# gyhandy/Neural-Sim-NeRF

Measured on AMD Instinct MI355X. Metric: Mray-samples/sec at 400x400, 64+128 samples, 8x256 MLP, higher is better.
Workload: dtype f16x2

## Files before the change

neural_sim_nerf_amd/csrc/nsr_h2.inc:

```
constexpr int kStreamSlabsH2Bwd = 146;


typedef _Float16 f16x8 __attribute__((ext_vector_type(8)));
typedef _Float16 f16x2 __attribute__((ext_vector_type(2)));
typedef float f32x2 __attribute__((ext_vector_type(2)));

struct H2 { u32x4 hi, lo; };

constexpr float kH2Max = 65504.0f * (1.0f - 1.0f / 4096.0f);

struct H2Job {
  float xa, xb, m;
  unsigned hi;
  float ra, rb;
};
__device__ __forceinline__ void h2_stage0(H2Job& q) {
  asm("v_fma_mixlo_f16 %0, %1, %2, 0" : "=v"(q.hi) : "v"(q.xa), "v"(q.m));
}
__device__ __forceinline__ void h2_stage1(H2Job& q, float& amax) {
  asm("v_fma_mixhi_f16 %0, %1, %2, 0" : "+v"(q.hi) : "v"(q.xb), "v"(q.m));
  asm("v_max3_f32 %0, %0, |%1|, |%2|" : "+v"(amax) : "v"(q.xa), "v"(q.xb));
}
__device__ __forceinline__ void h2_stage2(H2Job& q) {
  asm("v_fma_mix_f32 %0, %1, %2, -%3 op_sel:[0,0,0] op_sel_hi:[0,0,1]" : "=v"(q.ra) : "v"(q.xa), "v"(q.m), "v"(q.hi));
  asm("v_fma_mix_f32 %0, %1, %2, -%3 op_sel:[0,0,1] op_sel_hi:[0,0,1]" : "=v"(q.rb) : "v"(q.xb), "v"(q.m), "v"(q.hi));
}
__device__ __forceinline__ void h2_stage3(const H2Job& q, int j, H2& r) {
  const f16x2 lo = __builtin_convertvector(f32x2{q.ra, q.rb}, f16x2);
  r.hi[j] = q.hi;
  r.lo[j] = __builtin_bit_cast(unsigned, lo);
}
__device__ __forceinline__ void split_pair_h2(float xa, float xb, float m, int j, H2& r, float& amax) {
  H2Job q{xa, xb, m, 0u, 0.0f, 0.0f};
  h2_stage0(q); h2_stage1(q, amax); h2_stage2(q); h2_stage3(q, j, r);
}

__device__ __forceinline__ f32x16 mfma_h2(f32x4 a, u32x4 b, f32x16 c) {
  return __builtin_amdgcn_mfma_f32_32x32x16_f16(__builtin_bit_cast(f16x8, a), __builtin_bit_cast(f16x8, b), c, 0, 0, 0);
}

template <int C0>
__device__ __forceinline__ void ring_issue_dma(Ring& rg) {
  char* l = rg.smem + rg.pslot * kSlabBytes + rg.wave_lds;
  const int soff = rg.pnet_off + rg.pslab * kSlabBytes;
#ifndef NSR_EXP_NODMA
  __builtin_amdgcn_raw_ptr_buffer_load_lds(rg.rsrc, (__attribute__((address_space(3))) void*)l, 16, rg.lane_off, soff,
                                           C0 * 1024, 0);
  __builtin_amdgcn_raw_ptr_buffer_load_lds(rg.rsrc, (__attribute__((address_space(3))) void*)l, 16, rg.lane_off, soff,
                                           (C0 + 1) * 1024, 0);
#endif
}
template <int C>
__device__ __forceinline__ void ring_issue_dma1(Ring& rg) {
  char* l = rg.smem + rg.pslot * kSlabBytes + rg.wave_lds;
  const int soff = rg.pnet_off + rg.pslab * kSlabBytes;
#ifndef NSR_EXP_NODMA
  __builtin_amdgcn_raw_ptr_buffer_load_lds(rg.rsrc, (__attribute__((address_space(3))) void*)l, 16, rg.lane_off, soff,
                                           C * 1024, 0);
#endif
}
template <int NS, int SLABS, int SLABS_BWD>
__device__ __forceinline__ void ring_issue_advance(Ring& rg) {
  rg.pslot = (rg.pslot + 1 == NS) ? 0 : rg.pslot + 1;
  const int nslab = rg.pslab + 1;
  const bool wrap = nslab == ((SLABS_BWD != SLABS && rg.pphase >= rg.pn1) ? SLABS_BWD : SLABS);
  rg.pslab = wrap ? 0 : nslab;
  const int nphase = (rg.pphase + 1 == rg.ppi) ? 0 : rg.pphase + 1;
  rg.pphase = wrap ? nphase : rg.pphase;
  const int net = rg.pphase < rg.pn0 ? 0 : (rg.pphase < rg.pn1 ? 1 : 2);
  rg.pnet_off = net * (int)rg.stride;
}

template <int NS, int SLABS, int SLABS_BWD>
__device__ __forceinline__ bool ring_issue_advance_a(Ring& rg) {
  rg.pslot = (rg.pslot + 1 == NS) ? 0 : rg.pslot + 1;
  const int nslab = rg.pslab + 1;
  const bool wrap = nslab == ((SLABS_BWD != SLABS && rg.pphase >= rg.pn1) ? SLABS_BWD : SLABS);
  rg.pslab = wrap ? 0 : nslab;
  return wrap;
}
__device__ __forceinline__ void ring_issue_advance_b(Ring& rg, bool wrap) {
  const int nphase = (rg.pphase + 1 == rg.ppi) ? 0 : rg.pphase + 1;
  rg.pphase = wrap ? nphase : rg.pphase;
  const int net = rg.pphase < rg.pn0 ? 0 : (rg.pphase < rg.pn1 ? 1 : 2);
  rg.pnet_off = net * (int)rg.stride;
}

template <int NS, int G, int NP, bool ACT_, bool ZH = false, bool ZL = false, int NACC>
__device__ __forceinline__ void step_h2(Ring& rg, f32x4 (&Acur)[4], f32x4 (&Anxt)[4], const H2& b, f32x16 (&acc)[NACC],
                                        int HB, int LB , int lane, H2Job (&job)[NP], int j0,
                                        H2& bn, float& amax) {
  const char* p = rg.smem + rg.cslot * kSlabBytes + (G + 1) * kStepBytes + lane * 16;
#ifdef NSR_EXP_H2_NOSPLIT
  constexpr bool ACT = false;
  if (ACT_) { bn = b; }
#else
  constexpr bool ACT = ACT_;
#endif
#ifdef NSR_EXP_H2_NOFRAG
#define NSR_H2_FRAG(i, off) do { } while (0)
#else
#define NSR_H2_FRAG(i, off) Anxt[i] = *(const f32x4*)(p + (off))
#endif
#ifdef NSR_EXP_NODMA
#define NSR_H2_DMA(C) do { } while (0)
#define NSR_H2_DMA1(C) do { } while (0)
#else
#define NSR_H2_DMA(C) ring_issue_dma<C>(rg)
#define NSR_H2_DMA1(C) ring_issue_dma1<C>(rg)
#endif
  const char* pn = nullptr;
  NSR_PIN();
  acc[HB] = mfma_h2(Acur[0], b.lo, ZH ? f32x16{0} : acc[HB]);
  NSR_PIN();
  if (G != 3) NSR_H2_FRAG(0, 0);
#if NSR_H2_SCHED == 3
  else NSR_H2_DMA1(3);
#endif
  if (ACT) for (int u = 0; u < NP; ++u) h2_stage0(job[u]);
  NSR_PIN();
  acc[HB + 1] = mfma_h2(Acur[1], b.lo, ZH ? f32x16{0} : acc[HB + 1]);
  NSR_PIN();
  if (G != 3) NSR_H2_FRAG(1, 1024);
  if (ACT) for (int u = 0; u < NP; ++u) h2_stage1(job[u], amax);
  if (G == 3) {
    NSR_PIN();
#ifdef NSR_EXP_NOVMWAIT
    asm volatile("s_waitcnt lgkmcnt(0)" ::: "memory");
#else
    asm volatile("s_waitcnt vmcnt(%0) lgkmcnt(0)" ::"n"(4 * (NS - 2)) : "memory");
#endif
#ifdef NSR_EXP_H2_HALFBARRIER
    if (rg.cslot & 1)
#endif
#ifndef NSR_EXP_NOBARRIER
    __builtin_amdgcn_s_barrier();
#endif
    rg.cslot = (rg.cslot + 1 == NS) ? 0 : rg.cslot + 1;
    pn = rg.smem + rg.cslot * kSlabBytes + lane * 16;
  }
  NSR_PIN();
  acc[LB] = mfma_h2(Acur[2], b.hi, ZL ? f32x16{0} : acc[LB]);
  NSR_PIN();
  if (G != 3) NSR_H2_FRAG(2, 2048);
  else { Anxt[0] = *(const f32x4*)(pn); if (NSR_H2_SCHED != 3) NSR_H2_DMA(0); }
  if (ACT) for (int u = 0; u < NP; ++u) h2_stage2(job[u]);
  NSR_PIN();
  acc[LB + 1] = mfma_h2(Acur[3], b.hi, ZL ? f32x16{0} : acc[LB + 1]);
  NSR_PIN();
  if (G != 3) NSR_H2_FRAG(3, 3072);
  else { Anxt[1] = *(const f32x4*)(pn + 1024); if (NSR_H2_SCHED != 3) NSR_H2_DMA(2); }
  if (ACT) for (int u = 0; u < NP; ++u) h2_stage3(job[u], j0 + u, bn);
  NSR_PIN();
  acc[HB] = mfma_h2(Acur[0], b.hi, acc[HB]);
  NSR_PIN();
#if NSR_H2_SCHED == 3
  if (G == 0) NSR_H2_DMA1(0);
  if (G == 1) NSR_H2_DMA1(1);
  if (G == 2) NSR_H2_DMA1(2);
#endif
#if NSR_H2_SCHED == 3
  bool wrapped = false;
  if (G == 3) { Anxt[2] = *(const f32x4*)(pn + 2048); wrapped = ring_issue_advance_a<NS, kStreamSlabs, kStreamSlabsH2Bwd>(rg); }
#else
  if (G == 3) { Anxt[2] = *(const f32x4*)(pn + 2048); ring_issue_advance<NS, kStreamSlabs, kStreamSlabsH2Bwd>(rg); }
#endif
  NSR_PIN();
  acc[HB + 1] = mfma_h2(Acur[1], b.hi, acc[HB + 1]);
  NSR_PIN();
  if (G == 3) Anxt[3] = *(const f32x4*)(pn + 3072);
#if NSR_H2_SCHED == 3
  if (G == 3) ring_issue_advance_b(rg, wrapped);
#endif
#undef NSR_H2_DMA
#undef NSR_H2_DMA1
#undef NSR_H2_FRAG
}

struct H2Scale {
  float m[2];
  int split;
  __device__ __forceinline__ float operator()(int kb) const { return kb < split ? m[0] : m[1]; }
};

template <int NMO, int NKB, bool ZERO = false, int NACC, typename Src>
__device__ __forceinline__ void gemm_h2(Ring& rg, f32x4 (&A0)[4], f32x4 (&A1)[4], Src src, const H2Scale scale,
                                        f32x16 (&acc)[NACC], int lane, float& amax) {
  static_assert(NMO == 8 || NMO == 4 || NMO == 2, "8, 4 or 2 output blocks");
  static_assert((NKB * NMO) % 8 == 0, "a GEMM is a whole number of slabs");
  constexpr int SPB = NMO / 2;
  constexpr int NP = 4 / SPB;
  float am[2] = {0.0f, 0.0f};
  H2 b;
#pragma unroll
  for (int j = 0; j < 4; ++j) split_pair_h2(src(0, 2 * j), src(0, 2 * j + 1), scale(0), j, b, am[0 >= scale.split]);
#pragma unroll
  for (int kb = 0; kb < NKB; ++kb) {
    H2 bn;
    const bool more = kb + 1 < NKB;
    const int cls = more && (kb + 1 >= scale.split);
#pragma unroll
    for (int s = 0; s < SPB; ++s) {
      H2Job job[NP];
#pragma unroll
      for (int u = 0; u < NP; ++u) {
        const int j = NP * s + u;
        job[u] = H2Job{more ? src(kb + 1, 2 * j) : 0.0f, more ? src(kb + 1, 2 * j + 1) : 0.0f, more ? scale(kb + 1) : 0.0f, 0u, 0.0f, 0.0f};
      }
      const int g = (kb * SPB + s) & 3;
      const int hb = 2 * s, lb = NMO == 2 ? 0 : 2 * (s ^ 1);
      const bool zh = ZERO && kb == 0 && (s & 1) == 0, zl = ZERO && kb == 0 && (s & 1) == 0 && NMO != 2;
#define NSR_H2_STEP(GG, AC, AN, ACTV, ZHV, ZLV) \
  step_h2<kRingSlots, GG, NP, ACTV, ZHV, ZLV>(rg, AC, AN, b, acc, hb, lb, lane, job, NP * s, bn, am[ACTV ? cls : 0])
#define NSR_H2_STEP_Z(GG, AC, AN, ACTV)                              \
  do {                                                               \
    if (zh && zl) NSR_H2_STEP(GG, AC, AN, ACTV, true, true);         \
    else if (zh) NSR_H2_STEP(GG, AC, AN, ACTV, true, false);         \
    else NSR_H2_STEP(GG, AC, AN, ACTV, false, false);                \
  } while (0)
      if (more) {
        if (g == 0) NSR_H2_STEP_Z(0, A0, A1, true);
        if (g == 1) NSR_H2_STEP_Z(1, A1, A0, true);
        if (g == 2) NSR_H2_STEP_Z(2, A0, A1, true);
        if (g == 3) NSR_H2_STEP_Z(3, A1, A0, true);
      } else {
        if (g == 0) NSR_H2_STEP_Z(0, A0, A1, false);
        if (g == 1) NSR_H2_STEP_Z(1, A1, A0, false);
        if (g == 2) NSR_H2_STEP_Z(2, A0, A1, false);
        if (g == 3) NSR_H2_STEP_Z(3, A1, A0, false);
      }
#undef NSR_H2_STEP_Z
#undef NSR_H2_STEP
    }
    if (more) b = bn;
  }
  NSR_PIN();
  amax = __builtin_fmaxf(amax, __builtin_fmaxf(am[0] * scale.m[0], am[1] * scale.m[1]));
}
```

neural_sim_nerf_amd/csrc/nsr_kernels.hip:

```cpp
#include <hip/hip_runtime.h>
#include <stdint.h>
#include "nsr_device.h"

#if !defined(NSR_UNIT_F32) && !defined(NSR_UNIT_H2) && !defined(NSR_UNIT_B3) && !defined(NSR_UNIT_X16)
#define NSR_UNIT_F32 1
#define NSR_UNIT_H2 1
#define NSR_UNIT_B3 1
#define NSR_UNIT_X16 1
#endif
#ifndef NSR_UNIT_F32
#define NSR_UNIT_F32 0
#endif
#ifndef NSR_UNIT_H2
#define NSR_UNIT_H2 0
#endif
#ifndef NSR_UNIT_B3
#define NSR_UNIT_B3 0
#endif
#ifndef NSR_UNIT_X16
#define NSR_UNIT_X16 0
#endif
#define NSR_CAT_(a, b) a##b
#define NSR_CAT(a, b) NSR_CAT_(a, b)

namespace nsr {

__device__ __forceinline__ int opaque_v(int x) { asm volatile("" : "+v"(x)); return x; }
template <typename T>
__device__ __forceinline__ const T* opaque_s(const T* p) { asm volatile("" : "+s"(p)); return p; }

__device__ __forceinline__ long long uniform64(long long v) {
  const unsigned lo = __builtin_amdgcn_readfirstlane((unsigned)v);
  const unsigned hi = __builtin_amdgcn_readfirstlane((unsigned)((unsigned long long)v >> 32));
  return (long long)(((unsigned long long)hi << 32) | lo);
}

constexpr int kRing16 = 3;

struct Ring {
  char* smem;
  const char* base;
  long long stride;
  int lane_off;
  int wave_lds;
  int pslab;
  int pslot;
  int pphase;
  int ppi;
  int cslot;
  int pnet_off;
  int pn0, pn1;
  int dd;
  int pnet_next;
  __amdgpu_buffer_rsrc_t rsrc;
};

__device__ __forceinline__ void ring_init(Ring& rg, char* smem, const void* base, long long stride, int ppi, int wave,
                                          int lane) {
  rg.smem = smem;
  rg.base = (const char*)base;
  rg.stride = stride;
  rg.lane_off = wave * 4096 + lane * 16;
  rg.wave_lds = wave * 4096;
  rg.pslab = 0; rg.pslot = 0; rg.pphase = 0; rg.cslot = 0; rg.pnet_off = 0;
  rg.ppi = ppi;
  rg.pn0 = 1; rg.pn1 = 4;
  rg.dd = 0; rg.pnet_next = 0;
  rg.rsrc = __builtin_amdgcn_make_buffer_rsrc((void*)base, 0, 0x7fffffff, 0x00020000);
}

template <int NS = kRingSlots, int SLABS = kStreamSlabs, int SLABS_BWD = SLABS>
__device__ __forceinline__ void ring_issue(Ring& rg) {
  char* l = rg.smem + rg.pslot * kSlabBytes + rg.wave_lds;
#ifndef NSR_EXP_NODMA
  const int soff = rg.pnet_off + rg.pslab * kSlabBytes;
#define NSR_BUFDMA(C)                                                                                      \
  __builtin_amdgcn_raw_ptr_buffer_load_lds(rg.rsrc, (__attribute__((address_space(3))) void*)l, 16, rg.lane_off, \
                                           soff, (C) * 1024, 0)
  NSR_BUFDMA(0); NSR_BUFDMA(1); NSR_BUFDMA(2); NSR_BUFDMA(3);
#undef NSR_BUFDMA
#endif
  rg.pslot = (rg.pslot + 1 == NS) ? 0 : rg.pslot + 1;
  const int nslab = rg.pslab + 1;
  const bool wrap = nslab == ((SLABS_BWD != SLABS && rg.pphase >= rg.pn1) ? SLABS_BWD : SLABS);
  rg.pslab = wrap ? 0 : nslab;
  const int nphase = (rg.pphase + 1 == rg.ppi) ? 0 : rg.pphase + 1;
  rg.pphase = wrap ? nphase : rg.pphase;
  const int net = rg.pphase < rg.pn0 ? 0 : (rg.pphase < rg.pn1 ? 1 : 2);
  const int named = wrap ? rg.pnet_next : rg.pnet_off;
  rg.pnet_off = rg.dd ? named : net * (int)rg.stride;
}

__device__ __forceinline__ void ring_assert_uniform(Ring& rg) {
  rg.pslab = __builtin_amdgcn_readfirstlane(rg.pslab);
  rg.pslot = __builtin_amdgcn_readfirstlane(rg.pslot);
  rg.pphase = __builtin_amdgcn_readfirstlane(rg.pphase);
  rg.cslot = __builtin_amdgcn_readfirstlane(rg.cslot);
  rg.pnet_off = __builtin_amdgcn_readfirstlane(rg.pnet_off);
  rg.pnet_next = __builtin_amdgcn_readfirstlane(rg.pnet_next);
}

#ifndef NSR_H2_SCHED
#define NSR_H2_SCHED 3
#endif
constexpr int kH2RingLag = NSR_H2_SCHED == 3 ? 1 : 0;
template <int NS = kRingSlots, int SLABS = kStreamSlabs, int SLABS_BWD = SLABS, int LAG = 0>
__device__ __forceinline__ void ring_start(Ring& rg, f32x4 (&A0)[4], int lane) {
#pragma unroll 1
  for (int s = 0; s < NS - LAG; ++s) ring_issue<NS, SLABS, SLABS_BWD>(rg);
  asm volatile("s_waitcnt vmcnt(%0)" ::"n"(4 * (NS - LAG - 1)) : "memory");
  __builtin_amdgcn_s_barrier();
  const char* p = rg.smem + rg.cslot * kSlabBytes + lane * 16;
#pragma unroll
  for (int c = 0; c < 4; ++c) A0[c] = *(const f32x4*)(p + c * 1024);
}

template <int U>
__device__ __forceinline__ void ring_load_quarter(const Ring& rg, f32x4 (&A)[4], int lane) {
  const char* p = rg.smem + rg.cslot * kSlabBytes + U * kStepBytes + lane * 16;
#pragma unroll
  for (int c = 0; c < 4; ++c) A[c] = *(const f32x4*)(p + c * 1024);
}

template <int NS = kRingSlots>
__device__ __forceinline__ void ring_advance(Ring& rg, f32x4 (&A)[4], int lane) {
  asm volatile("s_waitcnt vmcnt(%0) lgkmcnt(0)" ::"n"(4 * (NS - 2)) : "memory");
#ifndef NSR_EXP_NOBARRIER
  __builtin_amdgcn_s_barrier();
#endif
  rg.cslot = (rg.cslot + 1 == NS) ? 0 : rg.cslot + 1;
  const char* p = rg.smem + rg.cslot * kSlabBytes + lane * 16;
#pragma unroll
  for (int c = 0; c < 4; ++c) A[c] = *(const f32x4*)(p + c * 1024);
}

#define NSR_MFMA(a, b, c) __builtin_amdgcn_mfma_f32_32x32x2f32((a), (b), (c), 0, 0, 0)
__device__ __forceinline__ f32x16 mfma_op(float a, float b, f32x16 c) { return __builtin_amdgcn_mfma_f32_32x32x2f32(a, b, c, 0, 0, 0); }
__device__ __forceinline__ f32x4 mfma_op(float a, float b, f32x4 c) { return __builtin_amdgcn_mfma_f32_16x16x4f32(a, b, c, 0, 0, 0); }

template <int NMO, int KK0, int KK1, bool ZERO = false, int NACC, typename BOp, typename AccT>
__device__ __forceinline__ void consume(const f32x4 (&A)[4], int step, BOp bop, AccT (&acc)[NACC]) {
#pragma unroll
  for (int kk = KK0; kk < KK1; ++kk)
#pragma unroll
    for (int c = 0; c < 4; ++c) {
      const int n = 4 * step + c, tq = n / NMO, mo = n % NMO;
      if (ZERO && tq == 0 && kk == 0) acc[mo] = mfma_op(A[c][kk], bop(4 * tq + kk), AccT{0});
      else acc[mo] = mfma_op(A[c][kk], bop(4 * tq + kk), acc[mo]);
    }
}

#define NSR_PIN() __builtin_amdgcn_sched_barrier(0)
#define NSR_SGB(mask, n) __builtin_amdgcn_sched_group_barrier((mask), (n), 0)
#define NSR_MASK_VALU 0x002
#define NSR_MASK_SALU 0x004
#define NSR_MASK_MFMA 0x008
#define NSR_MASK_VMEM 0x010
#define NSR_MASK_DSRD 0x100
template <int N_MFMA>
__device__ __forceinline__ void step_pattern() {
#pragma unroll
  for (int i = 0; i < N_MFMA; ++i) {
    NSR_SGB(NSR_MASK_MFMA, 1);
    NSR_SGB(NSR_MASK_DSRD, 1);
    NSR_SGB(NSR_MASK_VALU, 2);
  }
}
template <int N_MFMA>
__device__ __forceinline__ void step_pattern_dma() {
#pragma unroll
  for (int i = 0; i < N_MFMA; ++i) {
    NSR_SGB(NSR_MASK_MFMA, 1);
    NSR_SGB(NSR_MASK_DSRD, 1);
    NSR_SGB(NSR_MASK_VMEM, 1);
    NSR_SGB(NSR_MASK_SALU, 3);
    NSR_SGB(NSR_MASK_VALU, 2);
  }
}

template <int NMO, int NTQ, int NS = kRingSlots, bool ZERO = false, int NACC, typename BOp, typename AccT>
__device__ __forceinline__ void seg(Ring& rg, f32x4 (&A0)[4], f32x4 (&A1)[4], BOp bop, AccT (&acc)[NACC],
                                    int lane) {
  static_assert((NMO * NTQ) % 16 == 0, "a segment is a whole number of slabs");
#pragma unroll
  for (int s = 0; s < NMO * NTQ / 4; s += 4) {
    NSR_PIN(); ring_load_quarter<1>(rg, A1, lane); consume<NMO, 0, 4, ZERO>(A0, s, bop, acc);     step_pattern<16>();
    NSR_PIN(); ring_load_quarter<2>(rg, A0, lane); consume<NMO, 0, 4, ZERO>(A1, s + 1, bop, acc); step_pattern<16>();
    NSR_PIN(); ring_load_quarter<3>(rg, A1, lane); consume<NMO, 0, 4, ZERO>(A0, s + 2, bop, acc); step_pattern<16>();
    NSR_PIN(); consume<NMO, 0, 1, ZERO>(A1, s + 3, bop, acc);
    NSR_PIN(); ring_advance<NS>(rg, A0, lane);
    ring_issue<NS>(rg); consume<NMO, 1, 4, ZERO>(A1, s + 3, bop, acc); step_pattern_dma<12>();
    NSR_PIN();
  }
}

template <int NG>
struct BRegs16 {
  const f32x16 (&v)[NG];
  __device__ __forceinline__ float operator()(int t) const { return v[t >> 4][t & 15]; }
};
template <int N>
struct BArr {
  const float (&v)[N];
  __device__ __forceinline__ float operator()(int t) const { return v[t]; }
};
struct BViews {
  const f32x16 (&v)[8];
  const float (&ed)[16];
  __device__ __forceinline__ float operator()(int t) const { return t < 128 ? v[(t & 127) >> 4][t & 15] : ed[t & 15]; }
};

__device__ __forceinline__ int aux_half(int lane) { return opaque_v((lane >> 5) * 4); }

template <int NMO>
__device__ __forceinline__ void load_bias(const float* bias, int h4 , f32x16 (&acc)[NMO]) {
#pragma unroll
  for (int mo = 0; mo < NMO; ++mo)
#pragma unroll
    for (int rq = 0; rq < 4; ++rq) {
      f32x4 v = *(const f32x4*)(bias + (mo * 4 + rq) * 8 + h4);
      acc[mo][rq * 4 + 0] = v[0];
      acc[mo][rq * 4 + 1] = v[1];
      acc[mo][rq * 4 + 2] = v[2];
      acc[mo][rq * 4 + 3] = v[3];
    }
}

#include "nsr_b3.inc"
#include "nsr_h2.inc"

constexpr int kMlpF32 = 0;
constexpr int kMlpB3 = 1;
constexpr int kMlpH2 = 2;

template <int NMO>
__device__ __forceinline__ uint4 relu_mask(const f32x16 (&acc)[NMO]) {
  unsigned w[4] = {0u, 0u, 0u, 0u};
#pragma unroll
  for (int mo = 0; mo < NMO; ++mo)
#pragma unroll
    for (int r = 0; r < 16; ++r) {
      const int on = max(__float_as_int(acc[mo][r]), 0) - 1;
      w[mo >> 1] = __builtin_amdgcn_alignbit(w[mo >> 1], (unsigned)on, 31);
    }
  return make_uint4(w[0], w[1], w[2], w[3]);
}

__device__ __forceinline__ float enc_trig(float a, int k) {
  const double kMagic = 6755399441055744.0;
  const double t = (double)a * 0.63661977236758134308;
  const double tm = t + kMagic;
  const int n = __double2loint(tm) + k;
  const double f = t - (tm - kMagic);
  const float r = (float)(f * 1.57079632679489661923);
  const float z = r * r;
  float ps = __builtin_fmaf(-1.9515295891e-4f, z, 8.3321608736e-3f);
  ps = __builtin_fmaf(ps, z, -1.6666654611e-1f);
  ps = __builtin_fmaf(ps * z, r, r);
  float pc = __builtin_fmaf(2.443315711809948e-5f, z, -1.388731625493765e-3f);
  pc = __builtin_fmaf(pc, z, 4.166664568298827e-2f);
  pc = __builtin_fmaf(pc * z, z, __builtin_fmaf(-0.5f, z, 1.0f));
  const float v = (n & 1) ? pc : ps;
  return __uint_as_float(__float_as_uint(v) ^ ((unsigned)(n & 2) << 30));
}

__device__ __forceinline__ float enc_domain(float x, int nfreq) {
  return __builtin_fabsf(x) < ldexpf(1.0f, 25 - nfreq) ? x : __builtin_nanf("");
}

__device__ __forceinline__ float enc_poison(float px, float py, float pz, float vx, float vy, float vz) {
  const float a = (enc_domain(px, kMultires) * 0.0f + enc_domain(py, kMultires) * 0.0f) + enc_domain(pz, kMultires) * 0.0f;
  const float b = (enc_domain(vx, kMultiresViews) * 0.0f + enc_domain(vy, kMultiresViews) * 0.0f) +
                  enc_domain(vz, kMultiresViews) * 0.0f;
  return __builtin_fabsf(a + b);
}

template <bool CAPTURE, int MODE = kMlpF32>
__device__ __forceinline__ void mlp_pass(Ring& rg, const float* aux, f32x4 (&A0)[4], f32x4 (&A1)[4], int lane,
                                         float px, float py, float pz, float vx, float vy, float vz,
                                         float (&raw)[4], uint4* mask_dst = nullptr , int mask_tid = 0,
                                         long long* tp = nullptr ) {
#ifdef NSR_PHASE_TIMING
  long long tpl = clock64();
#define NSR_TP(i) do { if (tp) { const long long t_ = clock64(); tp[i] += t_ - tpl; tpl = t_; } } while (0)
#else
#define NSR_TP(i) do { } while (0)
#endif
  const int h = lane >> 5;
  const int h4 = aux_half(lane);
  const float poison = enc_poison(px, py, pz, vx, vy, vz);
  float e[32];
  float ed[16];
  {
    const float p[3] = {px, py, pz};
    const float v[3] = {vx, vy, vz};
#pragma unroll
    for (int L = 0; L < kMultires; ++L)
#pragma unroll
      for (int ax = 0; ax < 3; ++ax) e[3 * L + ax] = enc_trig(enc_domain(p[ax], kMultires) * (float)(1 << L), h);
#pragma unroll
    for (int L = 0; L < kMultiresViews; ++L)
#pragma unroll
      for (int ax = 0; ax < 3; ++ax) ed[3 * L + ax] = enc_trig(enc_domain(v[ax], kMultiresViews) * (float)(1 << L), h);
    e[30] = h ? pz : px;
    e[31] = h ? 0.0f : py;
    ed[12] = h ? vz : vx;
    ed[13] = h ? 0.0f : vy;
    ed[14] = 0.0f;
    ed[15] = 0.0f;
  }

  f32x16 acc[8];
  f32x16 in[8];
  auto enc_src = [&](int kb, int i) { return e[(8 * kb + i) & 31]; };
  auto in_src = [&](int kb, int i) { return in[(kb >> 1) & 7][8 * (kb & 1) + i]; };
  constexpr bool B3 = MODE == kMlpB3;
  constexpr bool H2M = MODE == kMlpH2;
  float amax = 0.0f;
  const float* h2s = aux + kAuxH2Scale;
  NSR_TP(0);
  load_bias<8>(aux + kAuxBias, h4, acc);
  NSR_TP(2);
  if constexpr (B3) gemm_b3<8, 2>(rg, A0, A1, enc_src, acc, lane);
  else if constexpr (H2M) gemm_h2<8, 4>(rg, A0, A1, enc_src, H2Scale{{h2s[0], 0.0f}, 4}, acc, lane, amax);
  else seg<8, 8>(rg, A0, A1, BArr<32>{e}, acc, lane);
  NSR_TP(1);
  if (CAPTURE) mask_dst[mask_tid] = relu_mask<8>(acc);
#pragma unroll
  for (int mo = 0; mo < 8; ++mo) in[mo] = relu16(acc[mo]);

  float alpha_part = 0.0f;
#pragma unroll 1
  for (int L = 1; L <= 8; ++L) {
    load_bias<8>(aux + kAuxBias + L * 256, h4, acc);
    NSR_TP(2);
    if (L == 5) {
      if constexpr (B3) gemm_b3<8, 2>(rg, A0, A1, enc_src, acc, lane);
      else if constexpr (H2M) gemm_h2<8, 4>(rg, A0, A1, enc_src, H2Scale{{h2s[9], 0.0f}, 4}, acc, lane, amax);
      else seg<8, 8>(rg, A0, A1, BArr<32>{e}, acc, lane);
      NSR_TP(1);
    }
    if (L == 8) {
      const float* wa = aux + kAuxWAlpha;
#pragma unroll
      for (int tq = 0; tq < 32; ++tq) {
        f32x4 w = *(const f32x4*)(wa + tq * 8 + h4);
#pragma unroll
        for (int kk = 0; kk < 4; ++kk)
          alpha_part = __builtin_fmaf(w[kk], in[(4 * tq + kk) >> 4][(4 * tq + kk) & 15], alpha_part);
      }
    }
    if constexpr (B3) gemm_b3<8, 8>(rg, A0, A1, in_src, acc, lane);
    else if constexpr (H2M) gemm_h2<8, 16>(rg, A0, A1, in_src, H2Scale{{h2s[L], 0.0f}, 16}, acc, lane, amax);
    else seg<8, 32>(rg, A0, A1, BRegs16<8>{in}, acc, lane);
    NSR_TP(1);
    if (CAPTURE && L < 8) mask_dst[L * 256 + mask_tid] = relu_mask<8>(acc);
    const int thr = (L == 8) ? (int)0x80000000 : 0;
#pragma unroll
    for (int mo = 0; mo < 8; ++mo) in[mo] = clamp_bits16(acc[mo], thr);
  }

  f32x16 av[4];
  load_bias<4>(aux + kAuxBiasV, h4, av);
  NSR_TP(2);
  if constexpr (B3) {
    auto v_src = [&](int kb, int i) {
      return kb < 16 ? in[(kb >> 1) & 7][8 * (kb & 1) + i] : (kb < 18 ? ed[(8 * (kb - 16) + i) & 15] : 0.0f);
    };
    gemm_b3<4, 5>(rg, A0, A1, v_src, av, lane);
  } else if constexpr (H2M) {
    auto v_src = [&](int kb, int i) { return kb < 16 ? in[(kb >> 1) & 7][8 * (kb & 1) + i] : ed[(8 * (kb - 16) + i) & 15]; };
    gemm_h2<4, 18>(rg, A0, A1, v_src, H2Scale{{h2s[10], h2s[11]}, 16}, av, lane, amax);
  } else {
    seg<4, 36>(rg, A0, A1, BViews{in, ed}, av, lane);
  }
  NSR_TP(1);
  if (CAPTURE) mask_dst[8 * 256 + mask_tid] = relu_mask<4>(av);

  float part[4] = {0.0f, 0.0f, 0.0f, alpha_part};
  if constexpr (H2M) {
    const float ov = amax > kH2Max ? __builtin_nanf("") : 0.0f;
    part[0] = part[1] = part[2] = ov;
    part[3] = alpha_part + ov;
  }
#pragma unroll
  for (int c = 0; c < 3; ++c) {
    const float* wr = aux + kAuxWRgb + c * 128;
#pragma unroll
    for (int mo = 0; mo < 4; ++mo)
#pragma unroll
      for (int rq = 0; rq < 4; ++rq) {
        f32x4 w = *(const f32x4*)(wr + (mo * 4 + rq) * 8 + h4);
#pragma unroll
        for (int ri = 0; ri < 4; ++ri)
          part[c] = __builtin_fmaf(w[ri], fmaxf(av[mo][rq * 4 + ri], 0.0f), part[c]);
      }
  }
#pragma unroll
  for (int c = 0; c < 4; ++c) {
    float other = __shfl_xor(part[c], 32);
    float lo_half = h ? other : part[c];
    float hi_half = h ? part[c] : other;
    raw[c] = ((lo_half + hi_half) + aux[(c < 3) ? (kAuxBRgb + c) : kAuxBAlpha]) + poison;
  }
  NSR_TP(3);
#undef NSR_TP
}

template <int NSS, int NFS>
struct ItemStateT {
  static constexpr int kNS = NSS, kNF = NFS;
  float tcoarse[NSS];
  float ufine[128];
  float ray[2][16];
  float zc[2][NSS];
  float rawc[2][NSS][4];
  float w0[2][NSS];
  float cdf[2][NSS];
  float zs[2][128];
  float zf[2][NFS];
  float rawf[2][NFS][4];
  float alpha[2][NFS];
  float wf[2][NFS];
  float tf[2][NFS];
  float om[2][NFS];
  float bwd_scratch[2][NFS][2];
  float psum[2][NFS / 32][12];
  float gnorm[2];
  float res[2][8];
};
typedef ItemStateT<64, 192> ItemState;
typedef ItemStateT<128, 256> ItemStateBig;
static_assert(sizeof(ItemState) == 23048, "the YCB-V layout is part of the shipped kernels' LDS budget");
template <int NS> struct ItemStateFor { typedef ItemState type; };
template <> struct ItemStateFor<128> { typedef ItemStateBig type; };

__device__ __forceinline__ float sigmoidf_(float x) { return 1.0f / (1.0f + expf(-x)); }

template <int S, int R = 2, int STRIDE = S, typename ST>
__device__ __forceinline__ void composite(ST& st, const float* z, float* raw, float* wout, float* tout, int tid,
                                          const float* noise = nullptr ,
                                          long long row0 = 0, int valid = R) {
  static_assert(S % 8 == 0, "scan is unrolled by 8");
  for (int idx = tid; idx < R * S; idx += 256) {
    const int r = idx / S, i = idx - r * S;
    const float* zr = z + r * STRIDE;
    float dist = (i < S - 1) ? (zr[i + 1] - zr[i]) : 1e10f;
    dist = dist * st.ray[r][11];
    float* q = raw + (r * STRIDE + i) * 4;
    if (noise) q[3] = q[3] + noise[(row0 + (r < valid ? r : 0)) * S + i];
    const float sigma = fmaxf(q[3], 0.0f);
    const float a = 1.0f - expf(-sigma * dist);
    st.alpha[r][i] = a;
    st.om[r][i] = (1.0f - a) + 1e-10f;
    q[0] = sigmoidf_(q[0]);
    q[1] = sigmoidf_(q[1]);
    q[2] = sigmoidf_(q[2]);
  }
  __syncthreads();
  if ((tid & 63) == 0 && tid < 64 * R) {
    const int r = tid >> 6;
    double T = 1.0;
#pragma unroll 1
    for (int i0 = 0; i0 < S; i0 += 8) {
      double f[8];
#pragma unroll
      for (int k = 0; k < 8; ++k) f[k] = (double)st.om[r][i0 + k];
#pragma unroll
      for (int k = 0; k < 8; ++k) {
        tout[r * STRIDE + i0 + k] = (float)T;
        T = T * f[k];
      }
    }
  }
  __syncthreads();
  if (tid < 64 * R) {
    const int r = tid >> 6, l = tid & 63;
    const float* zr = z + r * STRIDE;
    const float* q = raw + r * STRIDE * 4;
    float cr = 0.f, cg = 0.f, cb = 0.f, depth = 0.f, acc = 0.f;
#pragma unroll
    for (int i = l; i < S; i += 64) {
      const float w = st.alpha[r][i] * tout[r * STRIDE + i];
      wout[r * STRIDE + i] = w;
      cr = cr + w * q[i * 4 + 0];
      cg = cg + w * q[i * 4 + 1];
      cb = cb + w * q[i * 4 + 2];
      depth = depth + w * zr[i];
      acc = acc + w;
    }
#pragma unroll
    for (int m = 32; m >= 1; m >>= 1) {
      cr += __shfl_xor(cr, m); cg += __shfl_xor(cg, m); cb += __shfl_xor(cb, m);
      depth += __shfl_xor(depth, m); acc += __shfl_xor(acc, m);
    }
    if (l == 0) {
      const float qd = depth / acc;
      float disp;
      if (qd != qd) disp = qd;
      else disp = 1.0f / fmaxf(1e-10f, qd);
      if (st.ray[r][12] != 0.0f) {
        const float bg = 1.0f - acc;
        cr = cr + bg; cg = cg + bg; cb = cb + bg;
      }
      st.res[r][0] = cr; st.res[r][1] = cg; st.res[r][2] = cb;
      st.res[r][3] = disp; st.res[r][4] = acc; st.res[r][5] = depth;
    }
  }
  __syncthreads();
}

template <int R, int NI, int NS, typename ST, typename BinsFn>
__device__ __forceinline__ void sample_pdf_item_ns(ST& st, const float* ufine, const float* w, int wstride, BinsFn bins,
                                                   int64_t* inds_out, int64_t inds_stride, int tid, int valid_rays,
                                                   const float* u_rays, long long row0, int write_mask) {
  constexpr int NW = NS - 2, NC = NS - 1;
  constexpr int NVEC = NW / 8, SILP = NVEC / 4;
  for (int e = tid; e < R * NW; e += 256) {
    const int r = e / NW, i = e - r * NW;
    st.alpha[r][i] = (w + r * wstride)[i] + 1e-5f;
  }
  __syncthreads();
  if ((tid & 63) == 0 && tid < 64 * R) {
    const int r = tid >> 6;
    const float* x = st.alpha[r];
    float lanes[8];
#pragma unroll
    for (int j = 0; j < 8; ++j) {
      float ps[4] = {0.0f, 0.0f, 0.0f, 0.0f};
#pragma unroll
      for (int i = 0; i < SILP; ++i)
#pragma unroll
        for (int k = 0; k < 4; ++k) ps[k] = ps[k] + x[(i * 4 + k) * 8 + j];
#pragma unroll
      for (int v = SILP * 4; v < NVEC; ++v) ps[0] = ps[0] + x[v * 8 + j];
      lanes[j] = ((ps[0] + ps[1]) + ps[2]) + ps[3];
    }
    float total = 0.0f;
#pragma unroll
    for (int i = NVEC * 8; i < NW; ++i) total = total + x[i];
#pragma unroll
    for (int j = 0; j < 8; ++j) total = total + lanes[j];
    st.res[r][7] = total;
  }
  __syncthreads();
  for (int e = tid; e < R * NW; e += 256) {
    const int r = e / NW, i = e - r * NW;
    st.om[r][i] = st.alpha[r][i] / st.res[r][7];
  }
  __syncthreads();
  if ((tid & 63) == 0 && tid < 64 * R) {
    const int r = tid >> 6;
    double run = 0.0;
    st.cdf[r][0] = 0.0f;
#pragma unroll 1
    for (int i = 0; i < NW; ++i) { run = run + (double)st.om[r][i]; st.cdf[r][i + 1] = (float)run; }
  }
  __syncthreads();
  if (tid < 128 * R && (tid & 127) < NI) {
    const int r = tid >> 7, k = tid & 127;
    const float u = u_rays ? u_rays[(row0 + (r < valid_rays ? r : 0)) * 128 + k] : ufine[k];
    const float* cdf = st.cdf[r];
    int lo = 0, hi = NC;
    while (lo < hi) {
      const int mid = (lo + hi) >> 1;
      if (cdf[NSR_IDX(mid, NC)] <= u) lo = mid + 1; else hi = mid;
    }
    const int ind = lo;
    const int below = max(ind - 1, 0);
    const int above = min(ind, NC - 1);
    const float c0 = cdf[NSR_IDX(below, NC)], c1 = cdf[NSR_IDX(above, NC)];
    const float b0 = bins(r, NSR_IDX(below, NC)), b1 = bins(r, NSR_IDX(above, NC));
    float denom = c1 - c0;
    if (denom < 1e-5f) denom = 1.0f;
    const float t = (u - c0) / denom;
    st.zs[r][k] = b0 + t * (b1 - b0);
    if (inds_out && r < valid_rays && ((write_mask >> r) & 1)) inds_out[r * inds_stride + k] = (int64_t)ind;
  }
  __syncthreads();
}

template <int R = 2, int NI = 128, int NS = 64, typename ST, typename BinsFn>
__device__ __forceinline__ void sample_pdf_item(ST& st, const float* ufine ,
                                                const float* w , int wstride, BinsFn bins,
                                                int64_t* inds_out , int64_t inds_stride, int tid,
                                                int valid_rays, const float* u_rays = nullptr ,
                                                long long row0 = 0, int write_mask = 3 ) {
  if constexpr (NS != 64) {
    sample_pdf_item_ns<R, NI, NS>(st, ufine, w, wstride, bins, inds_out, inds_stride, tid, valid_rays, u_rays, row0, write_mask);
    return;
  }
  if (tid < 64 * R && (tid & 63) < 62) {
    const int r = tid >> 6, i = tid & 63;
    st.alpha[r][i] = (w + r * wstride)[i] + 1e-5f;
  }
  __syncthreads();
  if ((tid & 63) == 0 && tid < 64 * R) {
    const int r = tid >> 6;
    const float* x = st.alpha[r];
    float lanes[8];
#pragma unroll
    for (int j = 0; j < 8; ++j) {
      float p0 = ((x[j] + x[32 + j]) + x[40 + j]) + x[48 + j];
      lanes[j] = ((p0 + x[8 + j]) + x[16 + j]) + x[24 + j];
    }
    float total = 0.0f;
#pragma unroll
    for (int i = 56; i < 62; ++i) total = total + x[i];
#pragma unroll
    for (int j = 0; j < 8; ++j) total = total + lanes[j];
    st.res[r][7] = total;
  }
  __syncthreads();
  if (tid < 64 * R && (tid & 63) < 62) {
    const int r = tid >> 6, i = tid & 63;
    st.om[r][i] = st.alpha[r][i] / st.res[r][7];
  }
  __syncthreads();
  if ((tid & 63) == 0 && tid < 64 * R) {
    const int r = tid >> 6;
    double run = 0.0;
    st.cdf[r][0] = 0.0f;
#pragma unroll 1
    for (int i0 = 0; i0 < 56; i0 += 8) {
      double f[8];
#pragma unroll
      for (int k = 0; k < 8; ++k) f[k] = (double)st.om[r][i0 + k];
#pragma unroll
      for (int k = 0; k < 8; ++k) { run = run + f[k]; st.cdf[r][i0 + k + 1] = (float)run; }
    }
#pragma unroll
    for (int i = 56; i < 62; ++i) { run = run + (double)st.om[r][i]; st.cdf[r][i + 1] = (float)run; }
  }
  __syncthreads();
  if (tid < 128 * R && (tid & 127) < NI) {
    const int r = tid >> 7, k = tid & 127;
    const float u = u_rays ? u_rays[(row0 + (r < valid_rays ? r : 0)) * 128 + k] : ufine[k];
    const float* cdf = st.cdf[r];
    int lo = 0, hi = 63;
    while (lo < hi) {
      const int mid = (lo + hi) >> 1;
      if (cdf[NSR_IDX(mid, 63)] <= u) lo = mid + 1; else hi = mid;
    }
    const int ind = lo;
    const int below = max(ind - 1, 0);
    const int above = min(ind, 62);
    const float c0 = cdf[NSR_IDX(below, 63)], c1 = cdf[NSR_IDX(above, 63)];
    const float b0 = bins(r, NSR_IDX(below, 63)), b1 = bins(r, NSR_IDX(above, 63));
    float denom = c1 - c0;
    if (denom < 1e-5f) denom = 1.0f;
    const float t = (u - c0) / denom;
    st.zs[r][k] = b0 + t * (b1 - b0);
    if (inds_out && r < valid_rays && ((write_mask >> r) & 1)) inds_out[r * inds_stride + k] = (int64_t)ind;
  }
  __syncthreads();
}

template <int NI = 128, typename ST>
__device__ __forceinline__ float zstd_wave(const ST& st, int r, int lane) {
  const bool in0 = lane < NI, in1 = lane + 64 < NI;
  double s = (in0 ? (double)st.zs[r][lane] : 0.0) + (in1 ? (double)st.zs[r][lane + 64] : 0.0);
#pragma unroll
  for (int m = 32; m >= 1; m >>= 1) s += shfl_xor_f64(s, m);
  const double mean = s * (1.0 / NI);
  const double d0 = in0 ? (double)st.zs[r][lane] - mean : 0.0, d1 = in1 ? (double)st.zs[r][lane + 64] - mean : 0.0;
  double v = d0 * d0 + d1 * d1;
// ... 2302 lines not shown
```

Before: 277.3.

## Overlap ReLU clamp and next-layer bias load with the last GEMM k-block

Adds a specialised tail for the f16x2 GEMM. Its final k-block interleaves the MFMAs with the ReLU/clamp of finished accumulators into the next layer's inputs and with LDS loads of the next layer's bias into the accumulators. This hides the per-layer epilogue (clamp plus bias load) behind matrix-core latency instead of running it serially after each GEMM. The views layer reuses the preloaded bias. In exchange the schedule is hand-ordered, depends on the bias layout (guarded by a static_assert), and is only enabled for schedule 3 without capture.

After: 281.9, median of 6. 1.02x the previous value.

```diff
diff --git a/neural_sim_nerf_amd/csrc/nsr_h2.inc b/neural_sim_nerf_amd/csrc/nsr_h2.inc
--- a/neural_sim_nerf_amd/csrc/nsr_h2.inc
+++ b/neural_sim_nerf_amd/csrc/nsr_h2.inc
@@ -175,6 +175,80 @@
 #undef NSR_H2_DMA
 #undef NSR_H2_DMA1
 #undef NSR_H2_FRAG
+}
+
+struct H2Tail {
+  f32x16 (&acc)[8];
+  f32x16 (&in)[8];
+  int thr;
+  unsigned bias;
+  __device__ __forceinline__ void clamp(int k, int q) const {
+#pragma unroll
+    for (int r = 4 * q; r < 4 * q + 4; ++r) in[k][r] = __int_as_float(max(__float_as_int(acc[k][r]), thr));
+  }
+  __device__ __forceinline__ void load(int k, int rq) const {
+    const f32x4 v = *(const __attribute__((address_space(3))) f32x4*)(bias + (k * 4 + rq) * 32);
+    acc[k][rq * 4 + 0] = v[0];
+    acc[k][rq * 4 + 1] = v[1];
+    acc[k][rq * 4 + 2] = v[2];
+    acc[k][rq * 4 + 3] = v[3];
+  }
+};
+__device__ __forceinline__ unsigned h2_lds_base(const float* p, int h4) {
+  return (unsigned)opaque_v((int)(unsigned)(size_t)(const __attribute__((address_space(3))) float*)(p + h4));
+}
+
+template <int NS, typename Tail>
+__device__ __forceinline__ void tail_h2(Ring& rg, f32x4 (&A0)[4], f32x4 (&A1)[4], const H2& b, f32x16 (&acc)[8], int lane,
+                                        const Tail& t) {
+  const char* p = rg.smem + rg.cslot * kSlabBytes + lane * 16;
+#define NSR_T_MFMA(k, frag, bop) NSR_PIN(); acc[k] = mfma_h2(frag, b.bop, acc[k]); NSR_PIN()
+#define NSR_T_READ(dst, c) dst = *(const f32x4*)(p + (c) * 1024)
+  NSR_T_MFMA(0, A0[0], lo); NSR_T_READ(A1[0], 4);
+  NSR_T_MFMA(1, A0[1], lo); NSR_T_READ(A1[1], 6);
+  NSR_T_MFMA(2, A0[2], hi); NSR_T_READ(A1[2], 7);
+  NSR_T_MFMA(0, A0[0], hi); NSR_T_READ(A1[3], 8);
+  NSR_T_MFMA(1, A0[1], hi); ring_issue_dma1<0>(rg);
+  NSR_T_MFMA(2, A1[0], lo); NSR_T_READ(A0[2], 9);
+  NSR_T_MFMA(0, A1[1], hi); NSR_T_READ(A0[0], 5);
+  NSR_T_MFMA(1, A1[2], hi); NSR_T_READ(A0[1], 10);
+  NSR_T_MFMA(2, A1[0], hi); NSR_T_READ(A1[1], 14); t.clamp(0, 0); t.clamp(0, 1);
+  NSR_T_MFMA(3, A0[3], hi); NSR_T_READ(A1[2], 11); t.clamp(0, 2); t.clamp(0, 3);
+  NSR_T_MFMA(4, A1[3], lo); ring_issue_dma1<1>(rg); t.clamp(1, 0); t.clamp(1, 1);
+  NSR_T_MFMA(5, A0[2], lo); NSR_T_READ(A1[0], 12); t.clamp(1, 2); t.clamp(1, 3);
+  NSR_T_MFMA(3, A0[0], lo); t.clamp(2, 0); t.clamp(2, 1); t.load(0, 0); t.load(0, 1);
+  NSR_T_MFMA(4, A1[3], hi); t.clamp(2, 2); t.clamp(2, 3); t.load(0, 2); t.load(0, 3);
+  NSR_T_MFMA(6, A0[1], hi); t.load(1, 0); t.load(1, 1);
+  NSR_T_MFMA(3, A0[0], hi); NSR_T_READ(A1[3], 13);
+  NSR_T_MFMA(4, A1[1], hi); ring_issue_dma1<2>(rg);
+  NSR_T_MFMA(7, A1[2], hi); NSR_T_READ(A1[1], 15); t.clamp(3, 0); t.clamp(3, 1);
+  NSR_T_MFMA(5, A0[2], hi); ring_issue_dma1<3>(rg); t.clamp(3, 2); t.clamp(3, 3);
+  NSR_T_MFMA(6, A1[0], lo);
+#ifdef NSR_EXP_NOVMWAIT
+  asm volatile("s_waitcnt lgkmcnt(0)" ::: "memory");
+#else
+  asm volatile("s_waitcnt vmcnt(%0) lgkmcnt(0)" ::"n"(4 * (NS - 2)) : "memory");
+#endif
+#ifndef NSR_EXP_NOBARRIER
+  __builtin_amdgcn_s_barrier();
+#endif
+  rg.cslot = (rg.cslot + 1 == NS) ? 0 : rg.cslot + 1;
+  p = rg.smem + rg.cslot * kSlabBytes + lane * 16;
+  NSR_T_MFMA(7, A1[3], lo); NSR_T_READ(A0[0], 0); t.clamp(4, 0); t.clamp(4, 1);
+  NSR_T_MFMA(5, A1[1], hi); NSR_T_READ(A0[1], 1); t.clamp(4, 2); t.clamp(4, 3);
+  NSR_T_MFMA(6, A1[0], hi); NSR_T_READ(A0[2], 2);
+  const bool wrapped = ring_issue_advance_a<NS, kStreamSlabs, kStreamSlabsH2Bwd>(rg);
+  NSR_T_MFMA(7, A1[3], hi); NSR_T_READ(A0[3], 3);
+  ring_issue_advance_b(rg, wrapped);
+  NSR_PIN();
+  t.load(1, 2); t.load(1, 3);
+#pragma unroll
+  for (int k = 2; k < 8; ++k) {
+    if (k >= 5) { t.clamp(k, 0); t.clamp(k, 1); t.clamp(k, 2); t.clamp(k, 3); }
+    t.load(k, 0); t.load(k, 1); t.load(k, 2); t.load(k, 3);
+  }
+#undef NSR_T_READ
+#undef NSR_T_MFMA
 }
 
 struct H2Scale {
@@ -237,3 +311,33 @@
   NSR_PIN();
   amax = __builtin_fmaxf(amax, __builtin_fmaxf(am[0] * scale.m[0], am[1] * scale.m[1]));
 }
+
+template <int NKB, typename Src, typename Tail>
+__device__ __forceinline__ void gemm_h2_tail(Ring& rg, f32x4 (&A0)[4], f32x4 (&A1)[4], Src src, const H2Scale scale,
+                                             f32x16 (&acc)[8], int lane, float& amax, const Tail tail) {
+  static_assert(NKB > 1, "the last block is not the first");
+  float am[2] = {0.0f, 0.0f};
+  H2 b;
+#pragma unroll
+  for (int j = 0; j < 4; ++j) split_pair_h2(src(0, 2 * j), src(0, 2 * j + 1), scale(0), j, b, am[0 >= scale.split]);
+#pragma unroll
+  for (int kb = 0; kb + 1 < NKB; ++kb) {
+    H2 bn;
+    const int cls = kb + 1 >= scale.split;
+#pragma unroll
+    for (int s = 0; s < 4; ++s) {
+      H2Job job[1] = {H2Job{src(kb + 1, 2 * s), src(kb + 1, 2 * s + 1), scale(kb + 1), 0u, 0.0f, 0.0f}};
+      const int hb = 2 * s, lb = 2 * (s ^ 1);
+#define NSR_H2_STEP(GG, AC, AN) step_h2<kRingSlots, GG, 1, true, false, false>(rg, AC, AN, b, acc, hb, lb, lane, job, s, bn, am[cls])
+      if (s == 0) NSR_H2_STEP(0, A0, A1);
+      if (s == 1) NSR_H2_STEP(1, A1, A0);
+      if (s == 2) NSR_H2_STEP(2, A0, A1);
+      if (s == 3) NSR_H2_STEP(3, A1, A0);
+#undef NSR_H2_STEP
+    }
+    b = bn;
+  }
+  tail_h2<kRingSlots>(rg, A0, A1, b, acc, lane, tail);
+  NSR_PIN();
+  amax = __builtin_fmaxf(amax, __builtin_fmaxf(am[0] * scale.m[0], am[1] * scale.m[1]));
+}
diff --git a/neural_sim_nerf_amd/csrc/nsr_kernels.hip b/neural_sim_nerf_amd/csrc/nsr_kernels.hip
--- a/neural_sim_nerf_amd/csrc/nsr_kernels.hip
+++ b/neural_sim_nerf_amd/csrc/nsr_kernels.hip
@@ -318,21 +318,31 @@
   constexpr bool H2M = MODE == kMlpH2;
   float amax = 0.0f;
   const float* h2s = aux + kAuxH2Scale;
+#if NSR_H2_SCHED == 3 && !defined(NSR_EXP_H2_NOFRAG) && !defined(NSR_EXP_H2_HALFBARRIER) && !defined(NSR_EXP_H2_NOSPLIT)
+  constexpr bool TAIL = H2M && !CAPTURE;
+#else
+  constexpr bool TAIL = false;
+#endif
+  static_assert(kAuxBiasV == kAuxBias + 9 * 256, "the views layer's bias follows feature_linear's: 'bias of layer L + 1' for L = 8");
   NSR_TP(0);
   load_bias<8>(aux + kAuxBias, h4, acc);
   NSR_TP(2);
   if constexpr (B3) gemm_b3<8, 2>(rg, A0, A1, enc_src, acc, lane);
+  else if constexpr (TAIL)
+    gemm_h2_tail<4>(rg, A0, A1, enc_src, H2Scale{{h2s[0], 0.0f}, 4}, acc, lane, amax, H2Tail{acc, in, 0, h2_lds_base(aux + kAuxBias + 256, h4)});
   else if constexpr (H2M) gemm_h2<8, 4>(rg, A0, A1, enc_src, H2Scale{{h2s[0], 0.0f}, 4}, acc, lane, amax);
   else seg<8, 8>(rg, A0, A1, BArr<32>{e}, acc, lane);
   NSR_TP(1);
   if (CAPTURE) mask_dst[mask_tid] = relu_mask<8>(acc);
-#pragma unroll
-  for (int mo = 0; mo < 8; ++mo) in[mo] = relu16(acc[mo]);
+  if constexpr (!TAIL) {
+#pragma unroll
+    for (int mo = 0; mo < 8; ++mo) in[mo] = relu16(acc[mo]);
+  }
 
   float alpha_part = 0.0f;
 #pragma unroll 1
   for (int L = 1; L <= 8; ++L) {
-    load_bias<8>(aux + kAuxBias + L * 256, h4, acc);
+    if constexpr (!TAIL) load_bias<8>(aux + kAuxBias + L * 256, h4, acc);
     NSR_TP(2);
     if (L == 5) {
       if constexpr (B3) gemm_b3<8, 2>(rg, A0, A1, enc_src, acc, lane);
@@ -351,17 +361,27 @@
       }
     }
     if constexpr (B3) gemm_b3<8, 8>(rg, A0, A1, in_src, acc, lane);
+    else if constexpr (TAIL)
+      gemm_h2_tail<16>(rg, A0, A1, in_src, H2Scale{{h2s[L], 0.0f}, 16}, acc, lane, amax,
+                       H2Tail{acc, in, (L == 8) ? (int)0x80000000 : 0, h2_lds_base(aux + kAuxBias + (L + 1) * 256, h4)});
     else if constexpr (H2M) gemm_h2<8, 16>(rg, A0, A1, in_src, H2Scale{{h2s[L], 0.0f}, 16}, acc, lane, amax);
     else seg<8, 32>(rg, A0, A1, BRegs16<8>{in}, acc, lane);
     NSR_TP(1);
     if (CAPTURE && L < 8) mask_dst[L * 256 + mask_tid] = relu_mask<8>(acc);
-    const int thr = (L == 8) ? (int)0x80000000 : 0;
-#pragma unroll
-    for (int mo = 0; mo < 8; ++mo) in[mo] = clamp_bits16(acc[mo], thr);
+    if constexpr (!TAIL) {
+      const int thr = (L == 8) ? (int)0x80000000 : 0;
+#pragma unroll
+      for (int mo = 0; mo < 8; ++mo) in[mo] = clamp_bits16(acc[mo], thr);
+    }
   }
 
   f32x16 av[4];
-  load_bias<4>(aux + kAuxBiasV, h4, av);
+  if constexpr (TAIL) {
+#pragma unroll
+    for (int mo = 0; mo < 4; ++mo) av[mo] = acc[mo];
+  } else {
+    load_bias<4>(aux + kAuxBiasV, h4, av);
+  }
   NSR_TP(2);
   if constexpr (B3) {
     auto v_src = [&](int kb, int i) {
```
